# TIXhjq/ML_Function

Measured on AMD Instinct MI355X. Metric: samples/sec fwd+bwd xDeepFM-CIN B=4096,F=39,K=16, higher is better.
Workload: dtype f32

## Files before the change

include/fil.h:

```cpp
#ifndef FIL_H_
#define FIL_H_

#include <stddef.h>
#include <stdint.h>

#ifdef __cplusplus
extern "C" {
#endif

typedef enum {
  FIL_OK = 0,
  FIL_ERR_ARG = -1,
  FIL_ERR_HIP = -2,
  FIL_ERR_WORKSPACE = -3,
  FIL_ERR_UNSUPPORTED = -4
} fil_status;

typedef enum { FIL_F32 = 0, FIL_BF16 = 1 } fil_dtype;

#define FIL_ABI_VERSION 216
int fil_version(void);
const char* fil_last_error(void);

int fil_profile_begin(const char* filter);
// ... 5 lines not shown
int fil_fm_pairs_fwd(const float* emb, float* pairs, int B, int F, int K, void* stream);
int fil_fm_pairs_bwd(const float* emb, const float* gpairs, float* demb, int B, int F, int K, void* stream);

int fil_dcn_fwd(const float* x, const float* w, const float* b, float* y, float* s, int B, int D, int L, void* stream);
size_t fil_dcn_bwd_workspace_bytes(int B, int D, int L);
int fil_dcn_bwd(const float* x, const float* w, const float* b, const float* s, const float* g, float* dx, float* dw,
                float* db, int B, int D, int L, void* workspace, size_t workspace_bytes, void* stream);

size_t fil_cin_saved_bytes(int B, int F, int K, int L, const int* H);
size_t fil_cin_fwd_workspace_bytes(int B, int F, int K, int L, const int* H);
size_t fil_cin_bwd_workspace_bytes(int B, int F, int K, int L, const int* H);
int fil_cin_grad_ready_points(int B, int F, int K, int L, const int* H, int mode, int* point);
int fil_cin_fwd(const float* x, const float* const* W, const float* const* bias, const float* dense_w,
                const float* dense_b, float* out, float* pooled, float* saved, int B, int F, int K, int L,
                const int* H, int output_dim, int mode, void* workspace, size_t workspace_bytes, void* stream);
int fil_cin_bwd(const float* x, const float* const* W, const float* const* bias, const float* dense_w,
                const float* pooled, const float* saved, const float* g, float* dx, float* const* dW,
                float* const* dbias, float* ddense_w, float* ddense_b, int B, int F, int K, int L, const int* H,
                int output_dim, int mode, void* const* grad_ready_events, void* workspace, size_t workspace_bytes,
                void* stream);
enum fil_cin_precision { FIL_CIN_PREC_DEFAULT = 0, FIL_CIN_PREC_BF16 = 1 };
int fil_cin_precision_used(int B, int F, int K, int L, const int* H, int mode, int precision);
int fil_cin_shortdx_used(int B, int F, int K, int L, const int* H, int output_dim, int mode, int precision);
int fil_cin_fwd_p(const float* x, const float* const* W, const float* const* bias, const float* dense_w,
                  const float* dense_b, float* out, float* pooled, float* saved, int B, int F, int K, int L,
                  const int* H, int output_dim, int mode, int precision, void* workspace, size_t workspace_bytes, void* stream);
int fil_cin_bwd_p(const float* x, const float* const* W, const float* const* bias, const float* dense_w,
                  const float* pooled, const float* saved, const float* g, float* dx, float* const* dW,
                  float* const* dbias, float* ddense_w, float* ddense_b, int B, int F, int K, int L, const int* H,
                  int output_dim, int mode, int precision, void* const* grad_ready_events, void* workspace, size_t workspace_bytes,
                  void* stream);

enum fil_cin_mode_bits { FIL_CIN_GENERAL = 1, FIL_CIN_BF16X3 = 2, FIL_CIN_MB2 = 4, FIL_CIN_NOSYM = 8, FIL_CIN_X_TRANSPOSED = 16,
                         FIL_CIN_NOTAIL = 32, FIL_CIN_TAIL_ALWAYS = 64, FIL_CIN_NOKSPLIT = 128, FIL_CIN_NOQTAIL = 256, FIL_CIN_NOQMERGE = 512 };
enum fil_precision { FIL_PREC_F32 = 0, FIL_PREC_F16_MFMA = 1 };
int fil_attn_plan(int F, int K, int H, int A, int precision, int* plan );
size_t fil_attn_fwd_workspace_bytes(int B, int F, int K, int H, int A);
size_t fil_attn_bwd_workspace_bytes(int B, int F, int K, int H, int A, int have_saved);
int fil_attn_fwd(const float* x, const float* Wq, const float* Wk, const float* Wr, const float* gamma,
                 const float* beta, float* y, float* res_out, float* av_out, float* rstd_out, int B, int F, int K, int H,
                 int A, float scale, float eps, int fuse_relu, int precision, int x_chunk, void* workspace,
                 size_t workspace_bytes, void* stream);
int fil_attn_bwd(const float* x, const float* Wq, const float* Wk, const float* Wr, const float* gamma,
                 const float* beta, const float* dy, const float* dres_in, const float* y_saved, const float* av_saved,
                 const float* rstd_saved, float* dx, float* dWq, float* dWk, float* dWr, float* dgamma, float* dbeta, int B, int F, int K, int H,
                 int A, float scale, float eps, int fuse_relu, int precision, int x_chunk, void* workspace,
// ... 394 lines not shown
```

ml_function_amd/_lib.py:

```python
import ctypes
import os
import re

_HERE = os.path.dirname(os.path.abspath(__file__))
def _lib_path():
    default = os.path.join(_HERE, "libfil_hip.so")
    alt = os.environ.get("FIL_LIB_PATH")
    if not alt:
        return default
    abl = os.path.realpath(os.path.join(_HERE, "..", "tools", "abl")) + os.sep
    if os.path.realpath(alt).startswith(abl):
        return alt
    import warnings
    warnings.warn("FIL_LIB_PATH=%s is outside %s: ignored, loading the in-tree libfil_hip.so" % (alt, abl))
    return default


LIB_PATH = _lib_path()
HEADER_PATH = os.path.join(_HERE, "..", "include", "fil.h")

FIL_F32, FIL_BF16 = 0, 1
FIL_ADAM_KERAS, FIL_ADAM_LAZY = 0, 1
FIL_ADAM_ROLL_STEP, FIL_ADAM_ROLL_SKIP, FIL_ADAM_ROLL_FLUSH = 0, 1, 2
FIL_OPT_ADAGRAD, FIL_OPT_FTRL = 1, 2
# ... 22 lines not shown
_F = _c.c_float
_L = _c.c_int64

SIGNATURES = {
    "fil_version": (_I, []),
    "fil_last_error": (_c.c_char_p, []),
    "fil_profile_begin": (_I, [_c.c_char_p]),
    "fil_profile_end": (_Z, [_c.c_char_p, _Z]),
    "fil_fm_fwd": (_I, [_P, _P, _P, _I, _I, _I, _I, _P]),
    "fil_fm_bwd": (_I, [_P, _P, _P, _P, _I, _I, _I, _I, _P]),
    "fil_fm_pairs_fwd": (_I, [_P, _P, _I, _I, _I, _P]),
    "fil_fm_pairs_bwd": (_I, [_P, _P, _P, _I, _I, _I, _P]),
    "fil_dcn_fwd": (_I, [_P, _P, _P, _P, _P, _I, _I, _I, _P]),
    "fil_dcn_bwd_workspace_bytes": (_Z, [_I, _I, _I]),
    "fil_dcn_bwd": (_I, [_P, _P, _P, _P, _P, _P, _P, _P, _I, _I, _I, _P, _Z, _P]),
    "fil_cin_saved_bytes": (_Z, [_I, _I, _I, _I, _P]),
    "fil_cin_fwd_workspace_bytes": (_Z, [_I, _I, _I, _I, _P]),
    "fil_cin_bwd_workspace_bytes": (_Z, [_I, _I, _I, _I, _P]),
    "fil_cin_grad_ready_points": (_I, [_I, _I, _I, _I, _P, _I, _P]),
    "fil_cin_fwd": (_I, [_P, _P, _P, _P, _P, _P, _P, _P, _I, _I, _I, _I, _P, _I, _I, _P, _Z, _P]),
    "fil_cin_bwd": (_I, [_P, _P, _P, _P, _P, _P, _P, _P, _P, _P, _P, _P, _I, _I, _I, _I, _P, _I, _I, _P, _P, _Z, _P]),
    "fil_cin_precision_used": (_I, [_I, _I, _I, _I, _P, _I, _I]),
    "fil_cin_shortdx_used": (_I, [_I, _I, _I, _I, _P, _I, _I, _I]),
    "fil_cin_fwd_p": (_I, [_P, _P, _P, _P, _P, _P, _P, _P, _I, _I, _I, _I, _P, _I, _I, _I, _P, _Z, _P]),
    "fil_cin_bwd_p": (_I, [_P, _P, _P, _P, _P, _P, _P, _P, _P, _P, _P, _P, _I, _I, _I, _I, _P, _I, _I, _I, _P, _P, _Z, _P]),
    "fil_attn_plan": (_I, [_I, _I, _I, _I, _I, _P]),
    "fil_attn_fwd_workspace_bytes": (_Z, [_I, _I, _I, _I, _I]),
    "fil_attn_bwd_workspace_bytes": (_Z, [_I, _I, _I, _I, _I, _I]),
    "fil_attn_fwd": (_I, [_P] * 10 + [_I, _I, _I, _I, _I, _F, _F, _I, _I, _I, _P, _Z, _P]),
    "fil_attn_bwd": (_I, [_P] * 17 + [_I, _I, _I, _I, _I, _F, _F, _I, _I, _I, _P, _Z, _P]),
    "fil_pattn_fwd": (_I, [_P, _P, _P, _P, _P, _I, _I, _I, _I, _I, _F, _I, _P]),
    "fil_pattn_bwd": (_I, [_P, _P, _P, _P, _P, _P, _P, _P, _I, _I, _I, _I, _I, _F, _I, _P]),
    "fil_embed_gather": (_I, [_P, _P, _P, _P, _P, _P, _I, _I, _I, _P]),
    "fil_embed_gather_dt": (_I, [_P, _P, _P, _P, _P, _P, _I, _I, _I, _I, _P]),
    "fil_embed_gather_xt": (_I, [_P, _P, _P, _P, _P, _P, _P, _I, _I, _I, _P]),
    "fil_embed_scatter_add": (_I, [_P, _P, _P, _P, _P, _I, _I, _I, _P]),
    "fil_embed_row_ids": (_I, [_P, _P, _P, _P, _P, _I, _I, _P]),
    "fil_embed_sort_fields": (_I, [_P, _P, _P, _P, _P, _P, _I, _I, _c.c_int64, _P]),
    "fil_embed_segment_sum": (_I, [_P, _P, _P, _P, _P, _P, _c.c_long, _I, _P]),
    "fil_embed_run_sum": (_I, [_P, _P, _P, _P, _c.c_long, _I, _P]),
    "fil_embed_run_sum_dt": (_I, [_P, _P, _P, _P, _c.c_long, _I, _I, _P]),
    "fil_embed_bag_fwd": (_I, [_P, _P, _P, _P, _c.c_int64, _P, _P, _P, _I, _I, _I, _I, _I, _P]),
    "fil_embed_bag_row_ids": (_I, [_P, _P, _P, _P, _c.c_int64, _P, _I, _I, _I, _P]),
    "fil_embed_bag_bwd_prep": (_I, [_P, _P, _P, _P, _P, _I, _I, _I, _I, _I, _P]),
    "fil_afm_plan": (_I, [_I, _I, _I, _I, _P]),
    "fil_afm_fwd": (_I, [_P, _P, _P, _P, _P, _P, _I, _I, _I, _I, _I, _P]),
# ... 242 lines not shown
```

ml_function_amd/csrc/cin.hip:

```cpp
#include "cin_layout.h"

namespace fil {

static const char* kFwdNames[kCinMaxL] = {"cin_fwd_l1", "cin_fwd_l2", "cin_fwd_l3", "cin_fwd_l4", "cin_fwd_l5", "cin_fwd_l6", "cin_fwd_l7", "cin_fwd_l8"};
static const char* kDwNames[kCinMaxL] = {"cin_bwd_dw_l1", "cin_bwd_dw_l2", "cin_bwd_dw_l3", "cin_bwd_dw_l4", "cin_bwd_dw_l5", "cin_bwd_dw_l6", "cin_bwd_dw_l7", "cin_bwd_dw_l8"};
static const char* kDzNames[kCinMaxL] = {"cin_bwd_dz_l1", "cin_bwd_dz_l2", "cin_bwd_dz_l3", "cin_bwd_dz_l4", "cin_bwd_dz_l5", "cin_bwd_dz_l6", "cin_bwd_dz_l7", "cin_bwd_dz_l8"};
static double gemm_flops(long M, int Hp, int F, int H) { return 2.0 * (double)M * Hp * F * H; }

static int launch_dw3(hipStream_t st, const DwPlan& p, const float* gT, int HS, const float* xT, const float* xpT, int xps, float* part,
                      long M, int F, int Hp, int H, int symD = 0, int xtra = 0) {
  const int items = p.blocks_x * p.splits * p.chunks;
  const dim3 grid((items + 7) / 8 * 8);
#define FIL_DW3(MBV, ONES) \
  hipLaunchKernelGGL((cin_dw3_kernel<MBV, ONES>), grid, dim3(kCinThreads), 0, st, gT, HS, xT, xpT, xps, part, (int)M, F, Hp, H, p.rows_per_split, \
                     p.blocks_x, p.chunks, items, symD, xtra)
  if (xT == nullptr) {
    if (p.MB == 2) FIL_DW3(2, true); else FIL_DW3(1, true);
  } else {
    if (p.MB == 2) FIL_DW3(2, false); else FIL_DW3(1, false);
  }
#undef FIL_DW3
  return p.splits;
}

// ... 22 lines not shown
struct CinPath {
  bool xt_in;
  bool general;
  bool tail;
  bool qtail;
  bool qmerge;
  bool qsplit;
  int qnp;
  CinTune tune;
  TailGeom tg;
  bool fwdq(const CinShape& s) const { return qmerge && knobs().fwdq != 0 && s.HS(0) == 128; }
};
static CinPath cin_path_of(const CinShape& s, int mode) {
  const CinTune tune(mode);
  return CinPath{(mode & FIL_CIN_X_TRANSPOSED) != 0, (mode & FIL_CIN_GENERAL) != 0, tail_used(s, mode), qtail_used(s, mode, tune), qmerge_used(s, mode, tune),
                 qsplit_used(s, mode, tune), (mode & kCinPrecBf16) != 0 ? 1 : 3, tune, tail_geom(s)};
}
static bool cin_ghat_used(const CinShape& s, const CinPath& p, int output_dim) {
  const bool headfold = output_dim == 1 && s.K <= 32 && (s.K & (s.K - 1)) == 0 && knobs().headfold != 0;
  const bool dz2 = knobs().dz2 != 0 && s.HS(0) / 2 == 64;
  return p.qmerge && p.fwdq(s) && !p.qsplit && headfold && dz2 && knobs().ghat != 0;
}
static bool cin_shortdx_used(const CinShape& s, const CinPath& p, int output_dim) { return cin_ghat_used(s, p, output_dim) && knobs().shortdx != 0; }
static int cin_precision_bits(const char* who, int mode, int precision, int* bits) {
  if (precision != FIL_CIN_PREC_DEFAULT && precision != FIL_CIN_PREC_BF16)
    return fail(FIL_ERR_ARG, "%s: precision %d (0 DEFAULT, 1 BF16)", who, precision);
  if (precision == FIL_CIN_PREC_BF16 && (mode & FIL_CIN_BF16X3) != 0)
    return fail(FIL_ERR_ARG, "%s: precision BF16 with mode bit BF16X3 (mode %d): two operand precisions", who, mode);
  *bits = precision == FIL_CIN_PREC_BF16 ? kCinPrecBf16 : 0;
  return FIL_OK;
}
static int cin_path(const char* who, const CinShape& s, int mode, int precision, CinPath* path) {
  if (mode < 0 || mode > 1023 || (mode & kCinRetiredBits) != 0)
    return fail(FIL_ERR_UNSUPPORTED, "%s: mode %d (bits: 1 general kernels, 2 BF16X3, 4 MB2, 8 NOSYM, 16 X_TRANSPOSED, 32 NOTAIL, 64 TAIL_ALWAYS, 128 NOKSPLIT, 256 NOQTAIL, 512 NOQMERGE)", who, mode);
  int bits = 0;
  if (int rc = cin_precision_bits(who, mode, precision, &bits)) return rc;
  *path = cin_path_of(s, mode | bits);
  return FIL_OK;
}
static int cin_ready_order(int L, const CinPath& p, int* slot, int* point) {
  int n = 0, pt = 0;
  slot[n] = L, point[n++] = pt;
  if (p.qmerge) slot[n] = 0, point[n++] = pt;
  ++pt;
  int l = L - 1;
  if (p.tail) {
// ... 45 lines not shown
}

extern "C" int fil_cin_grad_ready_points(int B, int F, int K, int L, const int* H, int mode, int* point) {
  CinShape s;
  if (int rc = check_shape("fil_cin_grad_ready_points", B, F, K, L, H, s)) return rc;
  if (point == nullptr || mode < 0 || mode > 1023) return fail(FIL_ERR_ARG, "fil_cin_grad_ready_points: point == NULL or mode %d out of range", mode);
  if ((mode & kCinRetiredBits) != 0) return fail(FIL_ERR_UNSUPPORTED, "fil_cin_grad_ready_points: mode %d holds a retired bit (2: the split-bf16 experiment)", mode);
  if (B == 0) {
    for (int i = 0; i <= L; ++i) point[i] = 0;
    return 1;
  }
  int slot[kCinMaxL + 1], pt[kCinMaxL + 1];
  const int n = cin_ready_order(L, cin_path_of(s, mode), slot, pt);
  for (int i = 0; i <= L; ++i) point[slot[i]] = pt[i];
  return n;
}

extern "C" int fil_cin_shortdx_used(int B, int F, int K, int L, const int* H, int output_dim, int mode, int precision) {
  CinShape s;
  if (int rc = check_shape("fil_cin_shortdx_used", B, F, K, L, H, s)) return rc;
  CinPath p;
  if (int rc = cin_path("fil_cin_shortdx_used", s, mode, precision, &p)) return rc;
  return B > 0 && cin_shortdx_used(s, p, output_dim) ? 1 : 0;
}

extern "C" int fil_cin_precision_used(int B, int F, int K, int L, const int* H, int mode, int precision) {
  CinShape s;
  if (int rc = check_shape("fil_cin_precision_used", B, F, K, L, H, s)) return rc;
  if (mode < 0 || mode > 1023 || (mode & kCinRetiredBits) != 0) return fail(FIL_ERR_UNSUPPORTED, "fil_cin_precision_used: mode %d", mode);
  int bits = 0;
  if (int rc = cin_precision_bits("fil_cin_precision_used", mode, precision, &bits)) return rc;
  if (bits == 0 || B == 0) return FIL_CIN_PREC_DEFAULT;
  return cin_path_of(s, mode | bits).qsplit ? FIL_CIN_PREC_BF16 : FIL_CIN_PREC_DEFAULT;
}

#define FIL_CIN_CHECK_ARG(cond)                                                          \
  do {                                                                                   \
    if (!(cond)) return ::fil::fail(FIL_ERR_ARG, "%s: bad argument: %s", c.who, #cond); \
  } while (0)
#define FIL_CIN_FWD_LAUNCHED() FIL_CHECK_LAUNCH_W("cin_fwd_impl")
#define FIL_CIN_BWD_LAUNCHED() FIL_CHECK_LAUNCH_W("cin_bwd_impl")

struct CinCall {
  const char* who;
  CinShape s;
  CinPath p;
// ... 371 lines not shown
  const CinSaved& sv = c.sv;
  const CinBwdWs& ws = c.ws;
  const int F = s.F, K = s.K, L = s.L, JT = s.JT(), LK = s.L * s.K, *H = s.H;
  const long M = s.M();
  const bool qsplit = c.p.qsplit;
  const float* xT = c.xT;
  hipStream_t st = c.st;
  const int p = tg.p, lL = L - 1, Hpp = tg.Hpp, Hq = tg.Hq, HS0 = s.HS(0);
  FIL_CIN_CHECK_ARG(c.bias && c.W[0] && c.W[p] && c.W[lL] && c.bias[p] && c.dW[0] && c.dW[p] && c.dW[lL] && c.dbias[0] && c.dbias[p] && c.dbias[lL]);
  const float* xpT = sv.maps[p - 1];
  const int xps = s.xps(p);
  const float* dPp = c.dPsrc + (size_t)p * K;
  const float* dPL = c.dPsrc + (size_t)lL * K;
  const float* dPprev = c.dPsrc + (size_t)(p - 1) * K;
  const double algo_tail = gemm_flops(M, Hpp, F, Hq) + gemm_flops(M, Hq, F, tg.HL);
  const double algo1 = gemm_flops(M, F, F, H[0]);
  const int symD = F / 2 + 1, Cl = F * symD;
  const int JTs = cin_jt_sym(F);
  const int periods = cin_dz_periods(F, JTs), tiles0 = cin_slot_tiles(F, JTs);
  const bool ghat = cin_ghat_used(s, c.p, c.output_dim);
  const CinBwdWs::Scratch v = ws.scratch(s, true, ghat);
  const float* G = ghat ? sv.R : ws.G[c.cur];
  const float* gsc = ghat ? c.g : nullptr;
  {
    ProfScope ps("cin_tail_a", st, (double)M * (2 * F + 3) * sizeof(float));
    const size_t sh = (size_t)256 * (F + 3 + (c.output_dim == 1 ? L : 0) + (ghat ? 1 : 0)) * sizeof(float);
    allow_lds(cin_qtail_xe_kernel<3>, sh);
    allow_lds(cin_qtail_xe_kernel<1>, sh);
    const int np = (int)std::min<long>(((long)tiles0 * 32 * HS0 + 255) / 256, 1024);
    const int nq2 = qsplit ? 2 * std::min(cdiv(tiles0 * 512, 256), 256) : 0;
    if (c.p.qnp == 1)
      hipLaunchKernelGGL(cin_qtail_xe_kernel<1>, dim3(c.ndc + np + nq2), dim3(kXeThreads), sh, st, xT, dPL, dPp, LK, K, v.xr, ws.dcpart, (int)M, F,
                         c.ndc, c.output_dim == 1 ? c.g : nullptr, c.dense_w, c.pooled, ws.dP, ws.hpart, LK, lL, p, c.W[0], ws.Wz, H[0], JTs, HS0, tiles0, np, sv.T,
                         Hpp, ws.Wzb1, ws.Wzb2, ghat ? 1 : 0);
    else
      hipLaunchKernelGGL(cin_qtail_xe_kernel<3>, dim3(c.ndc + np + nq2), dim3(kXeThreads), sh, st, xT, dPL, dPp, LK, K, v.xr, ws.dcpart, (int)M, F,
                         c.ndc, c.output_dim == 1 ? c.g : nullptr, c.dense_w, c.pooled, ws.dP, ws.hpart, LK, lL, p, c.W[0], ws.Wz, H[0], JTs, HS0, tiles0, np, sv.T,
                         Hpp, ws.Wzb1, ws.Wzb2, ghat ? 1 : 0);
  }
  FIL_CIN_BWD_LAUNCHED();
  {
    ProfScope ps("cin_last_bwd", st, 6.0 * (double)M * Hpp * F);
    if (cin_shortdx_used(s, c.p, c.output_dim))
      cin_launch_shortcut_dx(st, xpT, xps, sv.wsumP, dPp, LK, ws.dxT, (int)M, F, K, Hpp);
    else if (ghat)
      cin_launch_last_bwd2(st, JT, xT, xpT, xps, sv.wsumP, sv.wsnP, dPp, LK, nullptr, nullptr, HS0, ws.dxT, (int)M, F, K, Hpp);
    else
      cin_launch_last_bwd2(st, JT, xT, xpT, xps, sv.wsumP, sv.wsnP, dPp, LK, dPprev, ws.G[c.cur], HS0, ws.dxT, (int)M, F, K, Hpp, sv.R, HS0, dPL, ws.small);
  }
  FIL_CIN_BWD_LAUNCHED();
  int dw_parts = 0;
  {
    ProfScope ps("cin_bwd_dw_q", st, algo1 + algo_tail, gemm_flops(M, 1, Cl, H[0]) + gemm_flops(M, 1, Cl, Hpp));
    if (qsplit) {
      const DwqbPlan bp = cin_dwqb_plan(M, Cl + F, cu_count());
      cin_launch_dwq_b(st, c.p.qnp, bp, G, xpT, HS0, v.xr, v.XS, ws.part, (int)M, F, symD);
      dw_parts = bp.splits;
    } else {
      const bool f4 = knobs().dwfold4 != 0;
      const int Cw = Cl + F + (ghat ? 1 : 0);
      const DwqPlan dp = f4 ? cin_dwq_plan4(M, Cw, cu_count()) : cin_dwq_plan(M, Cw, cu_count());
#define FIL_DWQ(FOLDV, GHV) \
  hipLaunchKernelGGL((cin_dwq_kernel<kDwqDepth, FOLDV, GHV>), dim3((dp.wgs + 7) / 8 * 8), dim3(kDwqThreads), 0, st, G, xpT, HS0, v.xr, v.XS, ws.part, (int)M, F, \
                     symD, dp.rows_per_split, dp.splits, dp.ncol_full, dp.rem, dp.wgs_full, dp.wgs)
      if (ghat) {
        if (f4) FIL_DWQ(4, true); else FIL_DWQ(2, true);
// ... 340 lines not shown
  c.events = grad_ready_events;
  if (B == 0) {
    for (int l = 0; l < L; ++l) {
      (void)hipMemsetAsync(dW[l], 0, (size_t)c.s.Hp(l) * F * H[l] * sizeof(float), c.st);
      (void)hipMemsetAsync(dbias[l], 0, (size_t)H[l] * sizeof(float), c.st);
    }
    if (output_dim == 1) {
      (void)hipMemsetAsync(ddense_w, 0, (size_t)L * K * sizeof(float), c.st);
      (void)hipMemsetAsync(ddense_b, 0, sizeof(float), c.st);
    }
    for (int l = 0; l <= L; ++l) cin_record_ready(c, l);
    return FIL_OK;
  }
  FIL_CIN_CHECK_ARG(g && dx && saved && (x || !c.p.xt_in));
  FIL_CIN_CHECK_ARG(output_dim != 1 || (dense_w && pooled && ddense_w && ddense_b));
  const size_t need = bwd_ws_bytes(c.s);
  if (workspace == nullptr || workspace_bytes < need) return fail(FIL_ERR_WORKSPACE, "fil_cin_bwd: workspace %zu < %zu bytes", workspace_bytes, need);
  c.x = x, c.W = W, c.bias = bias, c.dense_w = dense_w, c.pooled = pooled, c.g = g, c.output_dim = output_dim;
  c.dx = dx, c.dW = dW, c.dbias = dbias, c.ddense_w = ddense_w, c.ddense_b = ddense_b;
  LayoutCarver wsc(workspace), svc(saved);
  c.ws.lay_out(wsc, c.s);
  c.sv.lay_out(svc, c.s, c.p.tg, saved_form(c.p));
  c.xT = c.p.xt_in ? x : c.sv.xT;
  c.nblk = CinBwdWs::nblk(c.s), c.ncol = (int)CinBwdWs::ncol(c.s), c.ndc = (int)CinBwdWs::ndc(c.s);
  int point[kCinMaxL + 1];
  (void)cin_ready_order(L, c.p, c.ready_slot, point);
  if ((rc = cin_bwd_head(c)) != FIL_OK) return rc;
  if (c.p.qmerge) rc = cin_bwd_top_merged_q(c);
  else if (c.p.qtail) rc = cin_bwd_top_qtail(c);
  else if (c.p.tail) rc = cin_bwd_top_fused_tail(c);
  else if (!c.p.general) rc = cin_bwd_top_shortcut(c);
  else rc = cin_bwd_top_bcast(c);
  for (int l = c.ltop; l >= 0 && rc == FIL_OK; --l) rc = cin_bwd_general_layer(c, l);
  return rc != FIL_OK ? rc : cin_bwd_finish_dx(c);
}

extern "C" int fil_cin_bwd(const float* x, const float* const* W, const float* const* bias, const float* dense_w,
                           const float* pooled, const float* saved, const float* g, float* dx, float* const* dW,
                           float* const* dbias, float* ddense_w, float* ddense_b, int B, int F, int K, int L, const int* H,
                           int output_dim, int mode, void* const* grad_ready_events, void* workspace, size_t workspace_bytes,
                           void* stream) {
  return cin_bwd_impl("fil_cin_bwd", x, W, bias, dense_w, pooled, saved, g, dx, dW, dbias, ddense_w, ddense_b, B, F, K, L, H, output_dim, mode,
                      FIL_CIN_PREC_DEFAULT, grad_ready_events, workspace, workspace_bytes, stream);
}

extern "C" int fil_cin_bwd_p(const float* x, const float* const* W, const float* const* bias, const float* dense_w,
                             const float* pooled, const float* saved, const float* g, float* dx, float* const* dW,
// ... 7 lines not shown
```

ml_function_amd/csrc/cin_fwd.hip:

```cpp
#include "cin_kernels.h"
#include "cin_launch.h"
#include "cin_shortdx.h"

namespace fil {

template <int MB, int JT>
static void fwd3(hipStream_t st, dim3 grid, const float* xT, const float* xpT, int xps, const float* Wf, const float* bias,
                 float* xoutT, int HS, float* pool_part, int M, int F, int Hp, int H, const float* wsn, const float* bias_next,
                 int H_next, float* pool_next) {
  hipLaunchKernelGGL((cin_fwd3_kernel<MB, JT>), grid, dim3(kCinThreads), 0, st, xT, xpT, xps, Wf, bias, xoutT, HS, pool_part, M, F, Hp, H, wsn,
                     bias_next, H_next, pool_next);
}

void cin_launch_fwd3(hipStream_t st, int MB, int JT, dim3 grid, const float* xT, const float* xpT, int xps, const float* Wf,
                     const float* bias, float* xoutT, int HS, float* pool_part, int M, int F, int Hp, int H, const float* wsn,
                     const float* bias_next, int H_next, float* pool_next) {
#define FIL_F3(JTV)                                                                                                                      \
  case JTV:                                                                                                                              \
    if (MB == 2) fwd3<2, JTV>(st, grid, xT, xpT, xps, Wf, bias, xoutT, HS, pool_part, M, F, Hp, H, wsn, bias_next, H_next, pool_next);   \
    else fwd3<1, JTV>(st, grid, xT, xpT, xps, Wf, bias, xoutT, HS, pool_part, M, F, Hp, H, wsn, bias_next, H_next, pool_next);           \
    break;
  switch (JT) { FIL_F3(4) FIL_F3(8) FIL_F3(12) FIL_F3(16) FIL_F3(20) FIL_F3(24) FIL_F3(28) FIL_F3(32) }
#undef FIL_F3
}
// ... 39 lines not shown
                          const float* Radd, int HSr, const float* dPadd, float* colpart) {
#define FIL_LB(JTV) \
  case JTV: last_bwd2<JTV>(st, xT, xpT, xps, wsum, wsn, dP, ldp, dPprev, GprevT, HSp, dxT, M, F, K, Hp, Radd, HSr, dPadd, colpart); break;
  switch (JT) { FIL_LB(4) FIL_LB(8) FIL_LB(12) FIL_LB(16) FIL_LB(20) FIL_LB(24) FIL_LB(28) FIL_LB(32) }
#undef FIL_LB
}

template <int NT>
static void shortcut_dx(hipStream_t st, const float* xpT, int xps, const float* wsum, const float* dP, int ldp, float* dxT, int M, int F, int K, int Hp) {
  const size_t sh = cin_shortdx_lds_bytes(NT);
  if (sh > 48 * 1024)
    (void)hipFuncSetAttribute(reinterpret_cast<const void*>(cin_shortcut_dx_kernel<NT>), hipFuncAttributeMaxDynamicSharedMemorySize, (int)sh);
  hipLaunchKernelGGL((cin_shortcut_dx_kernel<NT>), dim3((M + 127) / 128), dim3(kCinThreads), sh, st, xpT, xps, wsum, dP, ldp, dxT, M, F, K, Hp);
}

void cin_launch_shortcut_dx(hipStream_t st, const float* xpT, int xps, const float* wsum, const float* dP, int ldp, float* dxT, int M, int F, int K,
                            int Hp) {
#define FIL_SDX(NTV) \
  case NTV: shortcut_dx<NTV>(st, xpT, xps, wsum, dP, ldp, dxT, M, F, K, Hp); break;
  switch ((F + 15) / 16) { FIL_SDX(1) FIL_SDX(2) FIL_SDX(3) FIL_SDX(4) }
#undef FIL_SDX
}

}
```

ml_function_amd/csrc/cin_launch.h:

```cpp
#pragma once
#include <hip/hip_runtime.h>

namespace fil {

inline int cin_jt_of(int F) { return ((F + 1) / 2 + 3) / 4 * 4; }

constexpr int kCinMaxFields = 64;
constexpr int cin_jt_sym(int F) { return ((F / 2 + 1 + 1) / 2 + 1) / 2 * 2; }
static_assert(cin_jt_sym(kCinMaxFields) <= 18, "the symmetric kernels' JT menu (2..18) must cover every legal field count");

inline int cin_x2_len(int F) { return F + 2 * cin_jt_sym(F); }
void cin_launch_fwd3_sym(hipStream_t st, int MB, int JT, dim3 grid, const float* xT, const float* x2T, int XL, const float* Wf, const float* bias,
                         float* xoutT, int HS, float* pool_part, int M, int F, int H, int ks = 1);

void cin_launch_fwd3(hipStream_t st, int MB, int JT, dim3 grid, const float* xT, const float* xpT, int xps, const float* Wf,
                     const float* bias, float* xoutT, int HS, float* pool_part, int M, int F, int Hp, int H,
                     const float* wsn = nullptr, const float* bias_next = nullptr, int H_next = 0, float* pool_next = nullptr);

void cin_launch_dz3(hipStream_t st, int MB, int JT, int NHMAX, dim3 grid, const float* gT, int HS, const float* Wz, const float* xT,
                    const float* xpT, int xps, const float* dPprev, int ldp, int K, float* GprevT, int HSp, float* gx0T, float* dxT,
                    int accumulate, int M, int F, int Hp, int H, int periods);

void cin_launch_last_bwd2(hipStream_t st, int JT, const float* xT, const float* xpT, int xps, const float* wsum, const float* wsn,
                          const float* dP, int ldp, const float* dPprev, float* GprevT, int HSp, float* dxT, int M, int F, int K, int Hp,
                          const float* Radd = nullptr, int HSr = 0, const float* dPadd = nullptr, float* colpart = nullptr);

void cin_launch_shortcut_dx(hipStream_t st, const float* xpT, int xps, const float* wsum, const float* dP, int ldp, float* dxT, int M, int F, int K,
                            int Hp);

void cin_launch_dz3_sym(hipStream_t st, int MB, int JT, int NHMAX, dim3 grid, const float* gT, int HS, const float* Wz, const float* xT,
                        float* gx0T, float* dxT, int accumulate, int M, int F, int H, int periods, int ks = 1);

inline int cin_gcd(int a, int b) { return b == 0 ? a : cin_gcd(b, a % b); }
inline int cin_dz_tiles_per_period(int JT) { return JT / cin_gcd(16, JT); }
inline int cin_dz_h_per_period(int JT) { return 16 * cin_dz_tiles_per_period(JT) / JT; }
inline int cin_dz_periods(int nh, int JT) { return (nh + cin_dz_h_per_period(JT) - 1) / cin_dz_h_per_period(JT); }
inline int cin_slot_tiles(int nh, int JT) { return cin_dz_periods(nh, JT) * cin_dz_tiles_per_period(JT) + 1; }

inline int cin_dz_sym_rows(int F, int JT) { return F > cin_dz_h_per_period(JT) + 2 * JT ? F : cin_dz_h_per_period(JT) + 2 * JT; }

inline bool cin_tail_supported(int F) { return F >= 1 && F <= 62; }
inline int cin_tail_ncb(int F) { return (F + 2 + 15) / 16; }
inline int cin_tail_jt4(int F) {
  const int v = (F + 3) / 4;
  return v == 11 ? 12 : (v == 13 ? 14 : v);
}
inline int cin_tail_nq(int F) { return ((F + 2) / 2 + 3) / 4; }
struct TailFwdArgs {
  const float *xT, *xpT;
  int xps;
  const float *Uf, *consts;
// ... 33 lines not shown
```

ml_function_amd/csrc/cin_layout.h:

```cpp
#pragma once
#include "cin_kernels.h"
#include "cin_tail.h"
#include "cin_launch.h"
#include "cin_qtail.h"
#include "cin_qsplit.h"
#include "cin_qmerge.h"

#include <stdlib.h>

namespace fil {

struct CinShape {
  int B, F, K, L;
  int H[kCinMaxL];
  int Hp(int l) const { return l == 0 ? F : H[l - 1]; }
  int HS(int l) const { return 128 * cdiv(H[l], 128); }
  int xps(int l) const { return l == 0 ? F : HS(l - 1); }
  long M() const { return (long)B * K; }
  int JT() const { return cin_jt_of(F); }
  int HSmax() const {
    int h = 0;
    for (int l = 0; l < L; ++l) h = std::max(h, HS(l));
    return h;
  }
};

static int check_shape(const char* fn, int B, int F, int K, int L, const int* H, CinShape& s) {
  if (B < 0 || F < 1 || K < 1 || L < 1 || H == nullptr) return fail(FIL_ERR_ARG, "%s: bad shape B=%d F=%d K=%d L=%d", fn, B, F, K, L);
  if (L > kCinMaxL) return fail(FIL_ERR_UNSUPPORTED, "%s: L=%d > %d", fn, L, kCinMaxL);
  if (F > kCinMaxFields) return fail(FIL_ERR_UNSUPPORTED, "%s: F=%d > %d fields", fn, F, kCinMaxFields);
  if ((long)B * K > (1L << 28)) return fail(FIL_ERR_UNSUPPORTED, "%s: B*K = %ld rows > 2^28 (row-split byte offsets of the dW kernel are 32-bit)", fn, (long)B * K);
  s.B = B; s.F = F; s.K = K; s.L = L;
  for (int l = 0; l < L; ++l) {
    if (H[l] < 1) return fail(FIL_ERR_ARG, "%s: H[%d]=%d", fn, l, H[l]);
    if (H[l] > kCinMaxH) return fail(FIL_ERR_UNSUPPORTED, "%s: H[%d]=%d > %d feature maps", fn, l, H[l], kCinMaxH);
    s.H[l] = H[l];
  }
  return FIL_OK;
}

static int chunks_of(int H) { return cdiv(H, 128); }
static int env_int(const char* name, int dflt) {
  const char* v = getenv(name);
  return v != nullptr && *v != 0 ? atoi(v) : dflt;
}
struct Knobs {
  int mb, sym, dw_mb, dw_splits, dz_mb, tail_splits, tail_settle, tail_dz_mode, ksplit, dzs_mb, qtail, qmerge, dz2, fwdq, headfold, packfold, dwfold4, ghat, shortdx;
};
static const Knobs& knobs() {
  static const Knobs k = {env_int("FIL_CIN_MB", 0), env_int("FIL_CIN_SYM", 1), env_int("FIL_CIN_DW_MB", 1), env_int("FIL_CIN_DW_SPLITS", 0),
                          env_int("FIL_CIN_DZ_MB", 1), env_int("FIL_CIN_TAIL_SPLITS", 0), env_int("FIL_CIN_TAIL_SETTLE", 0), env_int("FIL_CIN_TAIL_DZ_MODE", 0), env_int("FIL_CIN_KSPLIT", -1), env_int("FIL_CIN_DZS_MB", 0), env_int("FIL_CIN_QTAIL", 1), env_int("FIL_CIN_QMERGE", 1), env_int("FIL_CIN_DZ2", 1), env_int("FIL_CIN_FWDQ", 1), env_int("FIL_CIN_HEADFOLD", 1), env_int("FIL_CIN_PACKFOLD", 1), env_int("FIL_CIN_DWFOLD4", 1), env_int("FIL_CIN_GHAT", 1), env_int("FIL_CIN_SHORTDX", 1)};
  return k;
}
struct CinTune {
  int mb_forced;
  bool sym, no_ksplit;
  CinTune() : CinTune(0) {}
  explicit CinTune(int mode)
      : mb_forced((mode & FIL_CIN_MB2) ? 2 : knobs().mb), sym(knobs().sym != 0 && !(mode & FIL_CIN_NOSYM)), no_ksplit((mode & FIL_CIN_NOKSPLIT) != 0) {}
  int mb_rows(long M) const {
    if (mb_forced == 1 || mb_forced == 2) return mb_forced;
    return cdiv((int)std::min<long>(M, 1L << 30), 64) >= 768 ? 2 : 1;
  }
  int ksplit(long M) const {
    if (knobs().ksplit == 0 || no_ksplit) return 1;
    if (mb_rows(M) != 1) return 1;
    if (knobs().ksplit == 4) return 4;
    return cdiv((int)std::min<long>(M, 1L << 30), 32) <= 512 ? 4 : 1;
  }
};

struct DwPlan {
  int MB, blocks_x, splits, rows_per_split, chunks;
};
// ... 210 lines not shown
  template <class Taker>
  void lay_out(Taker& t, const CinShape& s) {
    const size_t M = (size_t)s.M(), LK = (size_t)s.L * s.K, HSmax = (size_t)s.HSmax();
    t.take(dP, (size_t)s.B * LK);
    t.take(G[0], M * HSmax);
    t.take(G[1], M * HSmax);
    t.take(part, dw_part_floats(s));
    t.take(small, std::max(ncol(s) * HSmax, (size_t)nblk(s) * (LK + 1)));
    const size_t cl = (size_t)std::max(s.Hp(s.L - 1), s.L == 3 ? s.H[0] : 0) * s.F;
    t.take(wsum, cl);
    t.take(vlast, cl);
    t.take(Wz, wz_floats(s));
    t.take(dxT, M * s.F);
    t.take(gx0T, M * s.F);
    t.take(dT, (size_t)s.F * s.F * kCinMaxH);
    t.take(dcpart, (ndc(s) + 1) * kQtConst);
    t.take(hpart, ndc(s) * (LK + 1));
    const size_t wzb = (size_t)cin_slot_tiles(s.F, cin_jt_sym(s.F)) * 8 * 3072 / sizeof(u32x4);
    t.take(Wzb1, wzb);
    t.take(Wzb2, wzb);
  }
  static int nblk(const CinShape& s) { return cdiv(std::max(1, s.B), kHeadChunk); }
  static size_t ncol(const CinShape& s) { return ((size_t)s.M() + kColRows - 1) / kColRows; }
  static size_t ndc(const CinShape& s) { return ((size_t)s.M() + 255) / 256; }
  struct Scratch {
    float *xr, *gxR, *dxR;
    int XS;
  };
  Scratch scratch(const CinShape& s, bool qmerge, bool ghat = false) const {
    const int XS = s.F + (qmerge ? (ghat ? 4 : 3) : 1);
    float* gxR = G[1] + (size_t)s.M() * XS;
    return Scratch{G[1], gxR, gxR + (size_t)s.M() * s.F, XS};
  }
};
static size_t bwd_ws_bytes(const CinShape& s) {
  LayoutSizer z;
  CinBwdWs().lay_out(z, s);
  return z.off;
}

}
```

ml_function_amd/csrc/cin_shortdx.h:

```cpp
#pragma once
#include "cin_kernels.h"

namespace fil {

constexpr int kSdxLd = 68;
constexpr int kSdxStage = 32 * kSdxLd;
constexpr int sdx_image_floats(int NT) { return 2 * NT * 4 * 64 * 4; }
inline size_t cin_shortdx_lds_bytes(int NT) { return (size_t)(sdx_image_floats(NT) + 4 * kSdxStage) * sizeof(float); }

template <int NT>
__global__ __launch_bounds__(256, 2) void cin_shortcut_dx_kernel(const float* __restrict__ xpT, int xps, const float* __restrict__ wsum,
                                                                const float* __restrict__ dP, int ldp, float* __restrict__ dxT, int M, int F,
                                                                int K, int Hp) {
  extern __shared__ __attribute__((aligned(16))) float smem[];
  const int tid = threadIdx.x, lane = tid & 63, wave = tid >> 6;
  const int c = lane & 15, g = lane >> 4;
  const int wrow0 = (blockIdx.x * 4 + wave) * 32;
  const long mq = min(wrow0 + (lane & 31), M - 1);
  const int bq = (int)(mq / K);
  const float dpv = dP[(long)bq * ldp + (int)(mq - (long)bq * K)];
  float wv[2 * NT][4];
#pragma unroll
  for (int q = 0; q < 2 * NT; ++q) {
    const int hh = q / NT, t = q - hh * NT;
    const int h0 = 64 * hh + 16 * g + 4 * wave, f = min(16 * t + c, F - 1);
#pragma unroll
    for (int e = 0; e < 4; ++e) wv[q][e] = wsum[min(h0 + e, Hp - 1) * F + f];
  }
  f32x4 v[16];
#pragma unroll
  for (int i = 0; i < 16; ++i) {
    const int hh = i >> 3;
    const int row = (lane >> 4) + 4 * (i & 7), col = 64 * hh + 4 * (lane & 15);
    v[i] = *reinterpret_cast<const f32x4*>(xpT + (long)min(wrow0 + row, M - 1) * xps + col);
    if (i == 7) __builtin_amdgcn_sched_barrier(0);
  }
  __builtin_amdgcn_sched_barrier(0);
  f32x4* img = reinterpret_cast<f32x4*>(smem);
#pragma unroll
  for (int q = 0; q < 2 * NT; ++q) {
    const int hh = q / NT, t = q - hh * NT;
    const int h0 = 64 * hh + 16 * g + 4 * wave;
    const bool fin = 16 * t + c < F;
    img[q * 256 + tid] = f32x4{fin && h0 < Hp ? wv[q][0] : 0.f, fin && h0 + 1 < Hp ? wv[q][1] : 0.f, fin && h0 + 2 < Hp ? wv[q][2] : 0.f,
                               fin && h0 + 3 < Hp ? wv[q][3] : 0.f};
  }
  __syncthreads();
  float* stg = smem + sdx_image_floats(NT) + wave * kSdxStage;
  f32x4 acc[2][NT];
#pragma unroll
  for (int rb = 0; rb < 2; ++rb)
#pragma unroll
    for (int t = 0; t < NT; ++t) acc[rb][t] = f32x4{0.f, 0.f, 0.f, 0.f};
#pragma unroll
  for (int hh = 0; hh < 2; ++hh) {
    {
      f32x4 a[2][4];
      __builtin_amdgcn_wave_barrier();
#pragma unroll
      for (int i = 0; i < 8; ++i) *reinterpret_cast<f32x4*>(stg + ((lane >> 4) + 4 * i) * kSdxLd + 4 * (lane & 15)) = v[8 * hh + i];
      __builtin_amdgcn_wave_barrier();
#pragma unroll
      for (int rb = 0; rb < 2; ++rb)
#pragma unroll
        for (int j = 0; j < 4; ++j) a[rb][j] = *reinterpret_cast<const f32x4*>(stg + (16 * rb + c) * kSdxLd + 16 * g + 4 * j);
#pragma unroll
      for (int s4 = 0; s4 < 4; ++s4) {
        f32x4 b[NT];
#pragma unroll
        for (int t = 0; t < NT; ++t) b[t] = img[((hh * NT + t) * 4 + s4) * 64 + lane];
#pragma unroll
        for (int e = 0; e < 4; ++e)
#pragma unroll
          for (int rb = 0; rb < 2; ++rb)
#pragma unroll
            for (int t = 0; t < NT; ++t) acc[rb][t] = __builtin_amdgcn_mfma_f32_16x16x4f32(a[rb][s4][e], b[t][e], acc[rb][t], 0, 0, 0);
      }
    }
  }
#pragma unroll
  for (int rb = 0; rb < 2; ++rb)
#pragma unroll
    for (int reg = 0; reg < 4; ++reg) {
      const int row = 16 * rb + 4 * g + reg, m = wrow0 + row;
      const float dpr = __shfl(dpv, row);
      if (m < M) {
#pragma unroll
        for (int t = 0; t < NT; ++t)
          if (16 * t + c < F) dxT[(long)m * F + 16 * t + c] = dpr * acc[rb][t][reg];
      }
    }
}

}
```

ml_function_amd/functional.py:

```python
import ctypes

import os

import time
import weakref

import torch

from . import _lib
from ._lib import FIL_BF16, FIL_F32, FilError, check, int_array, ptr, ptr_array, stream_ptr
from .optim import deferred_state


def _require_cuda(*tensors):
    for t in tensors:
        if t is not None and not t.is_cuda:
            raise FilError("ml_function_amd runs on the GPU only (got a %s tensor); there is no CPU fallback"
                           % t.device.type)


def _f32c(t):
    if t is None:
        return None
    if t.dtype != torch.float32:
# ... 847 lines not shown
def _cin_precision_code(precision):
    if precision not in _CIN_PRECISIONS:
        raise FilError("cin: precision must be one of %s, got %r" % (sorted(_CIN_PRECISIONS), precision))
    return _CIN_PRECISIONS[precision]


def cin_precision_used(B, F, K, H, mode=0, precision="bf16"):
    lib = _lib.load()
    code = _cin_precision_code(precision)
    rc = lib.fil_cin_precision_used(int(B), int(F), int(K), len(H), int_array(list(H)), int(mode), code)
    if rc < 0:
        raise FilError("fil_cin_precision_used: %s" % lib.fil_last_error().decode())
    return "bf16" if rc == CIN_PREC_BF16 else "f32"


def cin_shortdx_used(B, F, K, H, output_dim=1, mode=0, precision="f32"):
    lib = _lib.load()
    rc = lib.fil_cin_shortdx_used(int(B), int(F), int(K), len(H), int_array(list(H)), int(output_dim), int(mode), _cin_precision_code(precision))
    if rc < 0:
        raise FilError("fil_cin_shortdx_used: %s" % lib.fil_last_error().decode())
    return rc == 1


def cin_grad_ready_points(B, F, K, H, mode=0):
    lib = _lib.load()
    L = len(H)
    pts = (ctypes.c_int * (L + 1))()
    n = lib.fil_cin_grad_ready_points(int(B), int(F), int(K), L, int_array(list(H)), int(mode), pts)
    if n < 0:
        raise FilError("fil_cin_grad_ready_points: %s" % lib.fil_last_error().decode())
    return [int(v) for v in pts]


def cin_forward_raw(x, Ws, bs, dense_w, dense_b, output_dim=1, mode=0, xt=None, precision="f32"):
    lib = _lib.load()
    prec = _cin_precision_code(precision)
    B, F, K = x.shape
    if xt is not None:
        if tuple(xt.shape) != (B * K, F) or xt.dtype != torch.float32 or not xt.is_contiguous() or xt.device != x.device:
            raise FilError("cin: xt must be a contiguous float32 [B*K, F] = [%d, %d] tensor on %s" % (B * K, F, x.device))
        mode |= CIN_X_TRANSPOSED
    L = len(Ws)
    H = [int(w.shape[1]) for w in Ws]
    hp = F
    for l, w in enumerate(Ws):
        if tuple(w.shape) != (hp * F, H[l]) or tuple(bs[l].shape) != (H[l],):
# ... 757 lines not shown
```

Before: 5.910 million.

## Fold CIN qtail row prologue and Wz packing into shortcut-dx kernel

```diff
diff --git a/include/fil.h b/include/fil.h
--- a/include/fil.h
+++ b/include/fil.h
@@ -51,6 +51,7 @@
 enum fil_cin_precision { FIL_CIN_PREC_DEFAULT = 0, FIL_CIN_PREC_BF16 = 1 };
 int fil_cin_precision_used(int B, int F, int K, int L, const int* H, int mode, int precision);
 int fil_cin_shortdx_used(int B, int F, int K, int L, const int* H, int output_dim, int mode, int precision);
+int fil_cin_rowsfold_used(int B, int F, int K, int L, const int* H, int output_dim, int mode, int precision);
 int fil_cin_fwd_p(const float* x, const float* const* W, const float* const* bias, const float* dense_w,
                   const float* dense_b, float* out, float* pooled, float* saved, int B, int F, int K, int L,
                   const int* H, int output_dim, int mode, int precision, void* workspace, size_t workspace_bytes, void* stream);
diff --git a/ml_function_amd/_lib.py b/ml_function_amd/_lib.py
--- a/ml_function_amd/_lib.py
+++ b/ml_function_amd/_lib.py
@@ -68,6 +68,7 @@
     "fil_cin_bwd": (_I, [_P, _P, _P, _P, _P, _P, _P, _P, _P, _P, _P, _P, _I, _I, _I, _I, _P, _I, _I, _P, _P, _Z, _P]),
     "fil_cin_precision_used": (_I, [_I, _I, _I, _I, _P, _I, _I]),
     "fil_cin_shortdx_used": (_I, [_I, _I, _I, _I, _P, _I, _I, _I]),
+    "fil_cin_rowsfold_used": (_I, [_I, _I, _I, _I, _P, _I, _I, _I]),
     "fil_cin_fwd_p": (_I, [_P, _P, _P, _P, _P, _P, _P, _P, _I, _I, _I, _I, _P, _I, _I, _I, _P, _Z, _P]),
     "fil_cin_bwd_p": (_I, [_P, _P, _P, _P, _P, _P, _P, _P, _P, _P, _P, _P, _I, _I, _I, _I, _P, _I, _I, _I, _P, _P, _Z, _P]),
     "fil_attn_plan": (_I, [_I, _I, _I, _I, _I, _P]),
diff --git a/ml_function_amd/csrc/cin.hip b/ml_function_amd/csrc/cin.hip
--- a/ml_function_amd/csrc/cin.hip
+++ b/ml_function_amd/csrc/cin.hip
@@ -68,6 +68,7 @@
   return p.qmerge && p.fwdq(s) && !p.qsplit && headfold && dz2 && knobs().ghat != 0;
 }
 static bool cin_shortdx_used(const CinShape& s, const CinPath& p, int output_dim) { return cin_ghat_used(s, p, output_dim) && knobs().shortdx != 0; }
+static bool cin_rowsfold_used(const CinShape& s, const CinPath& p, int output_dim) { return cin_shortdx_used(s, p, output_dim) && knobs().rowsfold != 0; }
 static int cin_precision_bits(const char* who, int mode, int precision, int* bits) {
   if (precision != FIL_CIN_PREC_DEFAULT && precision != FIL_CIN_PREC_BF16)
     return fail(FIL_ERR_ARG, "%s: precision %d (0 DEFAULT, 1 BF16)", who, precision);
@@ -159,6 +160,14 @@
   CinPath p;
   if (int rc = cin_path("fil_cin_shortdx_used", s, mode, precision, &p)) return rc;
   return B > 0 && cin_shortdx_used(s, p, output_dim) ? 1 : 0;
+}
+
+extern "C" int fil_cin_rowsfold_used(int B, int F, int K, int L, const int* H, int output_dim, int mode, int precision) {
+  CinShape s;
+  if (int rc = check_shape("fil_cin_rowsfold_used", B, F, K, L, H, s)) return rc;
+  CinPath p;
+  if (int rc = cin_path("fil_cin_rowsfold_used", s, mode, precision, &p)) return rc;
+  return B > 0 && cin_rowsfold_used(s, p, output_dim) ? 1 : 0;
 }
 
 extern "C" int fil_cin_precision_used(int B, int F, int K, int L, const int* H, int mode, int precision) {
@@ -576,12 +585,13 @@
   const CinBwdWs::Scratch v = ws.scratch(s, true, ghat);
   const float* G = ghat ? sv.R : ws.G[c.cur];
   const float* gsc = ghat ? c.g : nullptr;
-  {
+  const bool rowsfold = cin_rowsfold_used(s, c.p, c.output_dim);
+  const int np = (int)std::min<long>(((long)tiles0 * 32 * HS0 + 255) / 256, 1024);
+  if (!rowsfold) {
     ProfScope ps("cin_tail_a", st, (double)M * (2 * F + 3) * sizeof(float));
     const size_t sh = (size_t)256 * (F + 3 + (c.output_dim == 1 ? L : 0) + (ghat ? 1 : 0)) * sizeof(float);
     allow_lds(cin_qtail_xe_kernel<3>, sh);
     allow_lds(cin_qtail_xe_kernel<1>, sh);
-    const int np = (int)std::min<long>(((long)tiles0 * 32 * HS0 + 255) / 256, 1024);
     const int nq2 = qsplit ? 2 * std::min(cdiv(tiles0 * 512, 256), 256) : 0;
     if (c.p.qnp == 1)
       hipLaunchKernelGGL(cin_qtail_xe_kernel<1>, dim3(c.ndc + np + nq2), dim3(kXeThreads), sh, st, xT, dPL, dPp, LK, K, v.xr, ws.dcpart, (int)M, F,
@@ -595,7 +605,10 @@
   FIL_CIN_BWD_LAUNCHED();
   {
     ProfScope ps("cin_last_bwd", st, 6.0 * (double)M * Hpp * F);
-    if (cin_shortdx_used(s, c.p, c.output_dim))
+    if (rowsfold)
+      cin_launch_shortcut_dx_rows(st, xpT, xps, sv.wsumP, ws.dxT, (int)M, F, K, Hpp,
+                                  SdxRows{xT, c.g, c.dense_w, c.pooled, v.xr, ws.dP, ws.dcpart, ws.hpart, kQtConst, c.W[0], ws.Wz, H[0], JTs, HS0, tiles0, np});
+    else if (cin_shortdx_used(s, c.p, c.output_dim))
       cin_launch_shortcut_dx(st, xpT, xps, sv.wsumP, dPp, LK, ws.dxT, (int)M, F, K, Hpp);
     else if (ghat)
       cin_launch_last_bwd2(st, JT, xT, xpT, xps, sv.wsumP, sv.wsnP, dPp, LK, nullptr, nullptr, HS0, ws.dxT, (int)M, F, K, Hpp);
@@ -982,7 +995,7 @@
   c.ws.lay_out(wsc, c.s);
   c.sv.lay_out(svc, c.s, c.p.tg, saved_form(c.p));
   c.xT = c.p.xt_in ? x : c.sv.xT;
-  c.nblk = CinBwdWs::nblk(c.s), c.ncol = (int)CinBwdWs::ncol(c.s), c.ndc = (int)CinBwdWs::ndc(c.s);
+  c.nblk = CinBwdWs::nblk(c.s), c.ncol = (int)CinBwdWs::ncol(c.s), c.ndc = (int)CinBwdWs::ndc(c.s, cin_rowsfold_used(c.s, c.p, output_dim));
   int point[kCinMaxL + 1];
   (void)cin_ready_order(L, c.p, c.ready_slot, point);
   if ((rc = cin_bwd_head(c)) != FIL_OK) return rc;
diff --git a/ml_function_amd/csrc/cin_fwd.hip b/ml_function_amd/csrc/cin_fwd.hip
--- a/ml_function_amd/csrc/cin_fwd.hip
+++ b/ml_function_amd/csrc/cin_fwd.hip
@@ -85,4 +85,21 @@
 #undef FIL_SDX
 }
 
+template <int NT>
+static void shortcut_dx_rows(hipStream_t st, const float* xpT, int xps, const float* wsum, float* dxT, int M, int F, int K, int Hp, const SdxRows& rows) {
+  const size_t sh = cin_shortdx_rows_lds_bytes(NT);
+  if (sh > 48 * 1024)
+    (void)hipFuncSetAttribute(reinterpret_cast<const void*>(cin_shortcut_dx_kernel<NT, SdxRows>), hipFuncAttributeMaxDynamicSharedMemorySize, (int)sh);
+  hipLaunchKernelGGL((cin_shortcut_dx_kernel<NT, SdxRows>), dim3((M + 127) / 128 + rows.npack), dim3(kCinThreads), sh, st, xpT, xps, wsum, nullptr, 3 * K, dxT, M, F,
+                     K, Hp, rows);
 }
+
+void cin_launch_shortcut_dx_rows(hipStream_t st, const float* xpT, int xps, const float* wsum, float* dxT, int M, int F, int K, int Hp,
+                                 const SdxRows& rows) {
+#define FIL_SDXR(NTV) \
+  case NTV: shortcut_dx_rows<NTV>(st, xpT, xps, wsum, dxT, M, F, K, Hp, rows); break;
+  switch ((F + 15) / 16) { FIL_SDXR(1) FIL_SDXR(2) FIL_SDXR(3) FIL_SDXR(4) }
+#undef FIL_SDXR
+}
+
+}
diff --git a/ml_function_amd/csrc/cin_launch.h b/ml_function_amd/csrc/cin_launch.h
--- a/ml_function_amd/csrc/cin_launch.h
+++ b/ml_function_amd/csrc/cin_launch.h
@@ -27,6 +27,16 @@
 
 void cin_launch_shortcut_dx(hipStream_t st, const float* xpT, int xps, const float* wsum, const float* dP, int ldp, float* dxT, int M, int F, int K,
                             int Hp);
+struct SdxRows {
+  const float *xT, *g, *dense_w, *pooled;
+  float *xe, *dP, *dcpart, *hpart;
+  int dcs;
+  const float* W0;
+  float* Wz;
+  int H0, JTs, HS0, tiles0, npack;
+};
+void cin_launch_shortcut_dx_rows(hipStream_t st, const float* xpT, int xps, const float* wsum, float* dxT, int M, int F, int K, int Hp,
+                                 const SdxRows& rows);
 
 void cin_launch_dz3_sym(hipStream_t st, int MB, int JT, int NHMAX, dim3 grid, const float* gT, int HS, const float* Wz, const float* xT,
                         float* gx0T, float* dxT, int accumulate, int M, int F, int H, int periods, int ks = 1);
diff --git a/ml_function_amd/csrc/cin_layout.h b/ml_function_amd/csrc/cin_layout.h
--- a/ml_function_amd/csrc/cin_layout.h
+++ b/ml_function_amd/csrc/cin_layout.h
@@ -45,11 +45,11 @@
   return v != nullptr && *v != 0 ? atoi(v) : dflt;
 }
 struct Knobs {
-  int mb, sym, dw_mb, dw_splits, dz_mb, tail_splits, tail_settle, tail_dz_mode, ksplit, dzs_mb, qtail, qmerge, dz2, fwdq, headfold, packfold, dwfold4, ghat, shortdx;
+  int mb, sym, dw_mb, dw_splits, dz_mb, tail_splits, tail_settle, tail_dz_mode, ksplit, dzs_mb, qtail, qmerge, dz2, fwdq, headfold, packfold, dwfold4, ghat, shortdx, rowsfold;
 };
 static const Knobs& knobs() {
   static const Knobs k = {env_int("FIL_CIN_MB", 0), env_int("FIL_CIN_SYM", 1), env_int("FIL_CIN_DW_MB", 1), env_int("FIL_CIN_DW_SPLITS", 0),
-                          env_int("FIL_CIN_DZ_MB", 1), env_int("FIL_CIN_TAIL_SPLITS", 0), env_int("FIL_CIN_TAIL_SETTLE", 0), env_int("FIL_CIN_TAIL_DZ_MODE", 0), env_int("FIL_CIN_KSPLIT", -1), env_int("FIL_CIN_DZS_MB", 0), env_int("FIL_CIN_QTAIL", 1), env_int("FIL_CIN_QMERGE", 1), env_int("FIL_CIN_DZ2", 1), env_int("FIL_CIN_FWDQ", 1), env_int("FIL_CIN_HEADFOLD", 1), env_int("FIL_CIN_PACKFOLD", 1), env_int("FIL_CIN_DWFOLD4", 1), env_int("FIL_CIN_GHAT", 1), env_int("FIL_CIN_SHORTDX", 1)};
+                          env_int("FIL_CIN_DZ_MB", 1), env_int("FIL_CIN_TAIL_SPLITS", 0), env_int("FIL_CIN_TAIL_SETTLE", 0), env_int("FIL_CIN_TAIL_DZ_MODE", 0), env_int("FIL_CIN_KSPLIT", -1), env_int("FIL_CIN_DZS_MB", 0), env_int("FIL_CIN_QTAIL", 1), env_int("FIL_CIN_QMERGE", 1), env_int("FIL_CIN_DZ2", 1), env_int("FIL_CIN_FWDQ", 1), env_int("FIL_CIN_HEADFOLD", 1), env_int("FIL_CIN_PACKFOLD", 1), env_int("FIL_CIN_DWFOLD4", 1), env_int("FIL_CIN_GHAT", 1), env_int("FIL_CIN_SHORTDX", 1), env_int("FIL_CIN_ROWSFOLD", 1)};
   return k;
 }
 struct CinTune {
@@ -306,7 +306,7 @@
   }
   static int nblk(const CinShape& s) { return cdiv(std::max(1, s.B), kHeadChunk); }
   static size_t ncol(const CinShape& s) { return ((size_t)s.M() + kColRows - 1) / kColRows; }
-  static size_t ndc(const CinShape& s) { return ((size_t)s.M() + 255) / 256; }
+  static size_t ndc(const CinShape& s, bool rows128 = true) { return ((size_t)s.M() + (rows128 ? 127 : 255)) / (rows128 ? 128 : 256); }
   struct Scratch {
     float *xr, *gxR, *dxR;
     int XS;
diff --git a/ml_function_amd/csrc/cin_shortdx.h b/ml_function_amd/csrc/cin_shortdx.h
--- a/ml_function_amd/csrc/cin_shortdx.h
+++ b/ml_function_amd/csrc/cin_shortdx.h
@@ -8,17 +8,52 @@
 constexpr int sdx_image_floats(int NT) { return 2 * NT * 4 * 64 * 4; }
 inline size_t cin_shortdx_lds_bytes(int NT) { return (size_t)(sdx_image_floats(NT) + 4 * kSdxStage) * sizeof(float); }
 
-template <int NT>
+constexpr int kSdxRowsSmall = 3 * 128 + 4 * 128 + 4 * 64 + 4;
+inline size_t cin_shortdx_rows_lds_bytes(int NT) { return cin_shortdx_lds_bytes(NT) + (size_t)kSdxRowsSmall * sizeof(float); }
+typedef float f32x4_a4 __attribute__((ext_vector_type(4), aligned(4)));
+template <class T>
+__device__ __forceinline__ const T& sdx_rows_of(const T& rows) { return rows; }
+
+template <int NT, class... Rows>
 __global__ __launch_bounds__(256, 2) void cin_shortcut_dx_kernel(const float* __restrict__ xpT, int xps, const float* __restrict__ wsum,
                                                                 const float* __restrict__ dP, int ldp, float* __restrict__ dxT, int M, int F,
-                                                                int K, int Hp) {
+                                                                int K, int Hp, Rows... rows) {
   extern __shared__ __attribute__((aligned(16))) float smem[];
+  constexpr bool ROWS = sizeof...(Rows) != 0;
   const int tid = threadIdx.x, lane = tid & 63, wave = tid >> 6;
   const int c = lane & 15, g = lane >> 4;
   const int wrow0 = (blockIdx.x * 4 + wave) * 32;
+  constexpr int NW = 2 * NT;
+  const int m0 = blockIdx.x * 128, rrow = tid & 127;
+  [[maybe_unused]] int nx = 0, nx4 = 0, rk = 0;
+  [[maybe_unused]] long rb = 0;
+  [[maybe_unused]] f32x4 xw[NW];
+  [[maybe_unused]] float xtail[3], gb = 0.f, dwv[3], plv[3];
+  if constexpr (ROWS) {
+    const SdxRows& ra = sdx_rows_of(rows...);
+    if (m0 >= M) {
+      const int nrb = (M + 127) / 128;
+      cin_pack_wz_sym_body(ra.W0, ra.Wz, F, ra.H0, ra.JTs, ra.HS0, ra.tiles0, blockIdx.x - nrb, gridDim.x - nrb);
+      return;
+    }
+    nx = min(128, M - m0) * F, nx4 = nx >> 2;
+    const float* src = ra.xT + (long)m0 * F;
+#pragma unroll
+    for (int u = 0; u < NW; ++u)
+      xw[u] = *reinterpret_cast<const f32x4_a4*>(nx4 > 0 ? src + 4 * min(tid + 256 * u, nx4 - 1) : xpT);
+#pragma unroll
+    for (int e = 0; e < 3; ++e) xtail[e] = src[min(4 * nx4 + e, nx - 1)];
+    const long m = min(m0 + rrow, M - 1);
+    rb = m / K, rk = (int)(m - rb * K);
+    gb = ra.g[rb];
+#pragma unroll
+    for (int l = 0; l < 3; ++l) dwv[l] = ra.dense_w[l * K + rk], plv[l] = ra.pooled[rb * (3 * K) + l * K + rk];
+    __builtin_amdgcn_sched_barrier(0);
+  }
   const long mq = min(wrow0 + (lane & 31), M - 1);
   const int bq = (int)(mq / K);
-  const float dpv = dP[(long)bq * ldp + (int)(mq - (long)bq * K)];
+  float dpv = 0.f;
+  if constexpr (!ROWS) dpv = dP[(long)bq * ldp + (int)(mq - (long)bq * K)];
   float wv[2 * NT][4];
 #pragma unroll
   for (int q = 0; q < 2 * NT; ++q) {
@@ -45,7 +80,88 @@
     img[q * 256 + tid] = f32x4{fin && h0 < Hp ? wv[q][0] : 0.f, fin && h0 + 1 < Hp ? wv[q][1] : 0.f, fin && h0 + 2 < Hp ? wv[q][2] : 0.f,
                                fin && h0 + 3 < Hp ? wv[q][3] : 0.f};
   }
+  float* small = smem + sdx_image_floats(NT) + 4 * kSdxStage;
+  float *dls = small, *dps = small + 128, *gs = small + 256, *hd = small + 384, *cs = small + 896;
+  if constexpr (ROWS) {
+    const SdxRows& ra = sdx_rows_of(rows...);
+    float* xs = smem + sdx_image_floats(NT);
+    const int rem = nx - 4 * nx4;
+#pragma unroll
+    for (int u = 0; u < NW; ++u) {
+      const int i = tid + 256 * u;
+      const f32x4 last = f32x4{rem > 0 ? xtail[0] : 0.f, rem > 1 ? xtail[1] : 0.f, rem > 2 ? xtail[2] : 0.f, 0.f};
+      reinterpret_cast<f32x4*>(xs)[i] = i < nx4 ? xw[u] : (i == nx4 ? last : f32x4{0.f, 0.f, 0.f, 0.f});
+    }
+    const bool live = m0 + rrow < M;
+    dls[rrow] = live ? gb * dwv[2] : 0.f;
+    dps[rrow] = live ? gb * dwv[1] : 0.f;
+    gs[rrow] = live ? gb : 0.f;
+#pragma unroll
+    for (int l = 0; l < 3; ++l) hd[rrow * 4 + l] = live ? gb * plv[l] : 0.f;
+    hd[rrow * 4 + 3] = live && rk == 0 ? gb : 0.f;
+    if (live && tid < 128) {
+#pragma unroll
+      for (int l = 0; l < 3; ++l) ra.dP[rb * (3 * K) + l * K + rk] = gb * dwv[l];
+    }
+    __syncthreads();
+    {
+      const int XE = F + 4, ne = min(128, M - m0) * XE, ne4 = ne >> 2;
+      float* dst = ra.xe + (long)m0 * XE;
+      const float rxe = 1.f / (float)XE;
+      for (int i4 = tid; i4 < ne4; i4 += 256) {
+        int rr = (int)(((float)(4 * i4) + 0.5f) * rxe);
+        int cc = 4 * i4 - rr * XE;
+        float e[4];
+#pragma unroll
+        for (int u = 0; u < 4; ++u) {
+          e[u] = cc < F ? xs[rr * F + cc] : cc == F ? 1.f : cc == F + 1 ? dls[rr] : cc == F + 2 ? dps[rr] : gs[rr];
+          if (++cc == XE) {
+            cc = 0;
+            ++rr;
+          }
+        }
+        reinterpret_cast<float4*>(dst)[i4] = make_float4(e[0], e[1], e[2], e[3]);
+      }
+      for (int i = 4 * ne4 + tid; i < ne; i += 256) {
+        const int rr = i / XE, cc = i - rr * XE;
+        dst[i] = cc < F ? xs[rr * F + cc] : cc == F ? 1.f : cc == F + 1 ? dls[rr] : cc == F + 2 ? dps[rr] : gs[rr];
+      }
+    }
+    {
+      const int f = lane, q = wave;
+      float t0 = 0.f, t1 = 0.f;
+      if (f < F) {
+        for (int rr = 32 * q; rr < 32 * q + 32; rr += 2) {
+          t0 += xs[rr * F + f] * dls[rr];
+          t1 += xs[(rr + 1) * F + f] * dls[rr + 1];
+        }
+      } else if (f < F + 2) {
+        const float* dv = f == F ? dls : dps;
+        for (int rr = 32 * q; rr < 32 * q + 32; rr += 2) {
+          t0 += dv[rr];
+          t1 += dv[rr + 1];
+        }
+      }
+      cs[q * 64 + f] = t0 + t1;
+    }
+    {
+      const int LK = 3 * K, k0 = m0 % K;
+      for (int j = tid; j <= LK; j += 256) {
+        float t = 0.f;
+        if (j < LK) {
+          const int l = j / K, k = j - l * K;
+          for (int rr = (k - k0 + K) % K; rr < 128; rr += K) t += hd[rr * 4 + l];
+        } else {
+          for (int rr = (K - k0) % K; rr < 128; rr += K) t += hd[rr * 4 + 3];
+        }
+        ra.hpart[(long)blockIdx.x * (LK + 1) + j] = t;
+      }
+    }
+  }
   __syncthreads();
+  if constexpr (ROWS) {
+    if (tid < F + 2) sdx_rows_of(rows...).dcpart[(long)blockIdx.x * sdx_rows_of(rows...).dcs + tid] = (cs[tid] + cs[64 + tid]) + (cs[128 + tid] + cs[192 + tid]);
+  }
   float* stg = smem + sdx_image_floats(NT) + wave * kSdxStage;
   f32x4 acc[2][NT];
 #pragma unroll
@@ -83,7 +199,7 @@
 #pragma unroll
     for (int reg = 0; reg < 4; ++reg) {
       const int row = 16 * rb + 4 * g + reg, m = wrow0 + row;
-      const float dpr = __shfl(dpv, row);
+      const float dpr = ROWS ? dps[32 * wave + row] : __shfl(dpv, row);
       if (m < M) {
 #pragma unroll
         for (int t = 0; t < NT; ++t)
diff --git a/ml_function_amd/functional.py b/ml_function_amd/functional.py
--- a/ml_function_amd/functional.py
+++ b/ml_function_amd/functional.py
@@ -893,6 +893,14 @@
     return rc == 1
 
 
+def cin_rowsfold_used(B, F, K, H, output_dim=1, mode=0, precision="f32"):
+    lib = _lib.load()
+    rc = lib.fil_cin_rowsfold_used(int(B), int(F), int(K), len(H), int_array(list(H)), int(output_dim), int(mode), _cin_precision_code(precision))
+    if rc < 0:
+        raise FilError("fil_cin_rowsfold_used: %s" % lib.fil_last_error().decode())
+    return rc == 1
+
+
 def cin_grad_ready_points(B, F, K, H, mode=0):
     lib = _lib.load()
     L = len(H)
```

Result: slower. 5.841 million (-1.2%).
